# dropbox/lepton

Measured on NVIDIA H100. Metric: JPEG MB/s encode+decode, higher is better.
Workload: dtype int16 coefficients / u8 probabilities (integer)

## Files before the change

lepton_b200/csrc/lep_decode_g2.cu:

```cuda
#include "lep_common.cuh"
#include "lep_predict.cuh"

namespace lepb200 {

struct G2Bool {
    unsigned long long value;
    uint32_t range;
    int valid;
    uint32_t next;
    const uint8_t* p;
    const uint8_t* end;
};

__device__ __forceinline__ uint32_t g2_load_word(const uint8_t* p, const uint8_t* end) {
    uint32_t w = 0;
    const long long rem = end - p;
    if (rem > 0) {
        w = __byte_perm(__ldg(reinterpret_cast<const uint32_t*>(p)), 0u, 0x0123u);
        if (rem < 4) w &= 0xffffffffu << (8 * (4 - (int)rem));
    }
    return w;
}
__device__ __forceinline__ void g2_refill(G2Bool& r) {
    r.value |= (unsigned long long)r.next << (32 - r.valid);
    r.valid += 32;
    r.p += 4;
    r.next = g2_load_word(r.p, r.end);
}
__device__ __forceinline__ void g2_init(G2Bool& r, const uint8_t* p, uint32_t len) {
    r.value = 0; r.valid = 0; r.range = 255;
    r.p = p; r.end = p + len;
    r.next = g2_load_word(r.p, r.end);
    g2_refill(r);
    const uint32_t split = (r.range * 128u + 128u) >> 8;
    const uint32_t bit = (uint32_t)(r.value >> 56) >= split;
    const uint32_t range = bit ? r.range - split : split;
    if (bit) r.value -= (unsigned long long)split << 56;
    const int shift = __clz(range) - 24;
    r.range = range << shift; r.value <<= shift; r.valid -= shift;
}

__device__ __forceinline__ uint32_t g2_bit(G2Bool& r, const uint32_t* rcp, uint32_t w, uint32_t& split) {
    const uint32_t prob = branch_prob(w, rcp);
    split = (r.range * prob + (256 - prob)) >> 8;
    if (r.valid < 32) g2_refill(r);
    return (uint32_t)(r.value >> 56) >= split;
}
__device__ __forceinline__ void g2_update(G2Bool& r, uint32_t split, uint32_t bit) {
    const uint32_t range = bit ? r.range - split : split;
    if (bit) r.value -= (unsigned long long)split << 56;
    const int shift = __clz(range) - 24;
    r.range = range << shift;
    r.value <<= shift;
    r.valid -= shift;
}
__device__ __forceinline__ uint32_t g2_model_word(uint32_t w, uint32_t bit) {
    const bool plain = (w & 0xffu) < 254u && (w >> 8) < 254u;
    return (plain ? w + (bit ? 0x100u : 1u) : branch_update(w, bit)) & 0xffffu;
}
__device__ __forceinline__ uint32_t g2_get(G2Bool& r, uint16_t* model, const uint32_t* rcp, uint32_t addr, uint32_t w) {
    uint32_t split;
    const uint32_t bit = g2_bit(r, rcp, w, split);
    g2_update(r, split, bit);
    model[addr] = (uint16_t)g2_model_word(w, bit);
    return bit;
}
#ifdef LEPB200_EMU
#define G2_EMU_BARRIER() __syncwarp()
#else
#define G2_EMU_BARRIER()
#endif

__device__ __forceinline__ uint32_t g2_half8(uint4 v, uint32_t i) {
    const uint32_t u = (i & 4u) ? ((i & 2u) ? v.w : v.z) : ((i & 2u) ? v.y : v.x);
    return (u >> ((i & 1u) << 4)) & 0xffffu;
}
__device__ __forceinline__ uint32_t g2_half4(uint2 v, uint32_t i) {
    return (((i & 2u) ? v.y : v.x) >> ((i & 1u) << 4)) & 0xffffu;
}
__device__ __forceinline__ uint16_t& g2_gword(uint16_t* model, uint32_t width, uint32_t addr) { return model[mi_offset(addr, 0, width)]; }
__device__ __forceinline__ uint32_t g2_unit(const uint16_t* model, uint32_t width, uint32_t addr) {
    return *reinterpret_cast<const uint32_t*>(model + mi_offset(addr, 0, width));
}
__device__ __forceinline__ uint4 g2_units4(const uint16_t* model, uint32_t width, uint32_t addr) {
    return make_uint4(g2_unit(model, width, addr), g2_unit(model, width, addr + 2), g2_unit(model, width, addr + 4),
                      g2_unit(model, width, addr + 6));
}
struct G2NzTop { uint32_t r5, r4; uint2 r3; uint4 r2; };
__device__ __forceinline__ G2NzTop g2_nz_top(const uint16_t* top, const uint16_t* model, uint32_t width, uint32_t rear) {
    G2NzTop v;
    v.r5 = top[nz7_row(5) - nz7_row(3)];
    v.r4 = *reinterpret_cast<const uint32_t*>(top + (nz7_row(4) - nz7_row(3)));
    v.r3 = *reinterpret_cast<const uint2*>(top);
    v.r2 = g2_units4(model, width, rear + nz7_row(2));
    return v;
}
__device__ __forceinline__ uint16_t* g2_word(uint16_t* hot, uint16_t* model, uint32_t width, uint32_t addr) {
    return addr < M_HOT ? hot + addr : &g2_gword(model, width, addr);
}
struct G2EdgeTree { uint32_t r2, r1; uint2 r0; };
__device__ __forceinline__ G2EdgeTree g2_edge_tree(const uint16_t* model, uint32_t width, uint32_t t) {
    G2EdgeTree v;
    v.r2 = model[mi_offset(t + (2 << 2), 0, width)];
    v.r1 = g2_unit(model, width, t + (1 << 2));
    v.r0 = make_uint2(g2_unit(model, width, t), g2_unit(model, width, t + 2));
    return v;
}

enum : int { G2_EXP = 0, G2_SIGN = 1, G2_THR = 2, G2_RES = 3 };

struct alignas(16) G2GroupSmem {
    int16_t blk[4][64];
    int32_t tmp[64];
    int16_t pix[64];
    int16_t ledge[8];
};
static_assert(sizeof(G2GroupSmem) == 512 + 256 + 128 + 16, "group scratch layout");

template <int G> struct G2Cfg {
    static constexpr int S = 32 / G;
    static constexpr int WARPS = (G >= 4) ? 4 : G;
    static constexpr int THREADS = WARPS * 32;
    static constexpr size_t HOT_BYTES = (size_t)WARPS * S * M_HOT * 2;
    static constexpr size_t SMEM_BYTES = 512 * 4 + 64 + 64 + 2 * 52 * 4 + sizeof(G2GroupSmem) * WARPS * S + HOT_BYTES;
    static_assert(SMEM_BYTES <= 113 * 1024, "two CTAs of the group kernel per SM");
};

template <int G> __device__ __forceinline__ int g2_sum(int v) {
#pragma unroll
    for (int d = 1; d < G; d <<= 1) v += __shfl_xor_sync(FULL, v, d);
    return v;
}
template <int G> __device__ __forceinline__ int g2_min(int v) {
#pragma unroll
    for (int d = 1; d < G; d <<= 1) v = min(v, __shfl_xor_sync(FULL, v, d));
    return v;
}
template <int G> __device__ __forceinline__ int g2_max(int v) {
#pragma unroll
    for (int d = 1; d < G; d <<= 1) v = max(v, __shfl_xor_sync(FULL, v, d));
    return v;
}
template <int G> __device__ __forceinline__ uint32_t g2_or(uint32_t v) {
#pragma unroll
    for (int d = 1; d < G; d <<= 1) v |= __shfl_xor_sync(FULL, v, d);
    return v;
}

__device__ __forceinline__ uint32_t g2_edge_info(int prior, int min_thr) {
    const int bsr = bitlen((uint32_t)min(iabs(prior), 1023));
    const int p16 = (int)(int16_t)prior;
    const int sctx = p16 == 0 ? 0 : (p16 > 0 ? 1 : 2);
    const int ctx_abs = iabs(prior) & 0xffff;
    return (uint32_t)bsr | ((uint32_t)sctx << 4) | ((uint32_t)min_thr << 6) | ((uint32_t)min(ctx_abs >> min_thr, 255) << 9);
}

template <int G>
__global__ void __launch_bounds__(G2Cfg<G>::THREADS)
lep_decode_g2_kernel(const ImageDesc* __restrict__ images, SegDesc* __restrict__ segs, int first, int count, const int* __restrict__ order,
                     int* __restrict__ work_counter, uint16_t* __restrict__ model_pool, uint8_t* __restrict__ row_pool, size_t row_pool_stride) {
    constexpr int S = G2Cfg<G>::S;
    constexpr int CPL = 64 / G;
    __shared__ uint32_t s_rcp[512];
    __shared__ uint8_t s_a2r[64];
    __shared__ uint8_t s_nzbin[64];
    __shared__ uint32_t s_eb[2][52];
    __shared__ G2GroupSmem s_grp[G2Cfg<G>::WARPS * S];
#ifndef LEPB200_EMU
    extern __shared__ uint4 s_hot[];
#else
    static uint4 s_hot[G2Cfg<G>::HOT_BYTES / 16];
#endif
    for (int i = threadIdx.x; i < 512; i += blockDim.x) s_rcp[i] = i < 2 ? 0u : (uint32_t)((0x100000000ull + i - 1) / i);
    for (int i = threadIdx.x; i < 64; i += blockDim.x) { s_a2r[i] = c_aligned_to_raster[i]; s_nzbin[i] = i < 50 ? c_nonzero_to_bin[i] : 0; }
    for (int i = threadIdx.x; i < 2 * 52; i += blockDim.x) {
        const int cc = i / 52, n = i % 52;
        s_eb[cc][n] = m_exp7(cc, n < 50 ? c_nonzero_to_bin[n] : 0, 0, 0);
    }
    __syncthreads();
    const int lane = lane_id();
    const int sub = lane & (G - 1);
    const int gbase = lane & ~(G - 1);
    const int slot = (blockIdx.x * G2Cfg<G>::WARPS + (threadIdx.x >> 5)) * S + lane / G;
    G2GroupSmem& gs = s_grp[(threadIdx.x >> 5) * S + lane / G];
    uint4* const hot4 = s_hot + (size_t)((threadIdx.x >> 5) * S + lane / G) * (M_HOT / 8);
    uint16_t* const hot = reinterpret_cast<uint16_t*>(hot4);
    uint16_t* const eoff = reinterpret_cast<uint16_t*>(gs.tmp);
    uint32_t* const einfo = reinterpret_cast<uint32_t*>(gs.tmp) + 32;
    uint8_t* rowbuf = row_pool + (size_t)slot * row_pool_stride;

    bool alive = false;
    bool exhausted = false;
    SegDesc* sdp = nullptr;
    const ImageDesc* gp = images;
    uint16_t* model = model_pool;
    uint32_t mwidth = 1;
    int seg_min_y = 0, seg_max_y = 0;
    bool seg_last = false;
    G2Bool br;
    br.value = 0; br.valid = 0; br.range = 255; br.next = 0; br.p = nullptr; br.end = nullptr;
    unsigned long long ndec = 0;
    uint32_t top_mask = 7u, index = 0;
    int bw0 = 0, bw1 = 0, bw2 = 0, nzs0 = 0, nzs1 = 0;
    size_t nz_base = 0;
    int c = 0, ci = 0, y = 0, w = 0, x = 0, q0 = 1, pc = 0, pa = 2, nz_left = 0;
    bool has_above = false, need_row = true;
    int16_t* rowp = nullptr;
    const int16_t* abovep = nullptr;
    const uint16_t* q = nullptr;
    int16_t* redge = nullptr;
    uint8_t* rnz = nullptr;
    const int32_t* icx = nullptr;
    const int32_t* icy = nullptr;
    const uint8_t* mthr = nullptr;
    uint32_t cnt_top = 0, cnt_rear = 0;
    G2NzTop nzt = {};
    bool cnt_ready = false;

    for (;;) {
        const bool want_job = !alive && !exhausted;
        const unsigned claim = __ballot_sync(FULL, want_job && sub == 0);
        if (claim) {
            const int leader = __ffs(claim) - 1;
            int job0 = 0;
            if (lane == leader) job0 = atomicAdd(work_counter, __popc(claim));
            job0 = __shfl_sync(FULL, job0, leader);
            if (want_job) {
                const int job = job0 + __popc(claim & ((1u << gbase) - 1u));
                if (job >= count) {
                    exhausted = true;
                } else {
                    const int sidx = order[first + job];
                    sdp = &segs[sidx];
                    if (sdp->status == ST_OK) {
                        gp = &images[sdp->image];
                        model = model_pool + mi_model((size_t)job, (size_t)count);
                        mwidth = mi_width((size_t)job, (size_t)count);
                        seg_min_y = sdp->min_y; seg_max_y = sdp->max_y; seg_last = sdp->is_last != 0;
                        g2_init(br, reinterpret_cast<const uint8_t*>(sdp->stream), sdp->cap);
                        ndec = 0; top_mask = 7u; index = 0;
                        bw0 = gp->bch[0]; bw1 = gp->ncmp > 1 ? gp->bch[1] : 0; bw2 = gp->ncmp > 2 ? gp->bch[2] : 0;
                        nz_base = (size_t)(bw0 + bw1 + bw2) * 16;
                        nzs0 = (bw0 + 15) & ~15; nzs1 = (bw1 + 15) & ~15;
                        need_row = true;
                        alive = true;
                        for (int i = sub; i < (int)(M_HOT / 8); i += G) hot4[i] = make_uint4(0u, 0u, 0u, 0u);
                    }
                }
            }
        }
        if (alive && need_row) {
            const ImageDesc& g = *gp;
            for (;;) {
                const RowSpec rs = row_spec_from_index(index++, g);
                if (rs.done || (rs.luma_y >= seg_max_y && !seg_last)) { alive = false; break; }
                if (rs.skip || rs.luma_y < seg_min_y) continue;
                c = rs.component; y = rs.curr_y;
                has_above = !((top_mask >> c) & 1u);
                top_mask &= ~(1u << c);
                ci = c == 0 ? 0 : 1;
                w = g.bch[c];
                rowp = reinterpret_cast<int16_t*>(g.plane[c]) + (size_t)y * w * 64;
                abovep = rowp - (size_t)w * 64;
                q = g.q[c];
                q0 = q[0];
                redge = reinterpret_cast<int16_t*>(rowbuf + (size_t)(c == 0 ? 0 : (c == 1 ? bw0 : bw0 + bw1)) * 16);
                rnz = rowbuf + nz_base + (c == 0 ? 0 : (c == 1 ? nzs0 : nzs0 + nzs1));
                icx = g.icos_x[c];
                icy = g.icos_y[c];
                mthr = g.min_thr[c];
                x = 0; pc = 0; pa = 2; nz_left = 0;
                need_row = false;
                break;
            }
            if (!alive && sub == 0) {
                sdp->status = ST_OK;
                sdp->len = (uint32_t)(br.p - reinterpret_cast<const uint8_t*>(sdp->stream));
                sdp->ndecisions_lo = (uint32_t)ndec;
                sdp->ndecisions_hi = (uint32_t)(ndec >> 32);
            }
        }
        if (__all_sync(FULL, exhausted)) break;

        const bool has_left = x > 0;
        int16_t* rcur = gs.blk[pc];
        const int16_t* rleft = gs.blk[pc ^ 1];
        int16_t* rabove = gs.blk[pa];
        const int16_t* raleft = gs.blk[pa ^ 1];
        uint32_t nd = 0;
        int nz = 0;

        if (alive) {
            if (has_above) {
                const uint32_t* src = reinterpret_cast<const uint32_t*>(abovep + (size_t)x * 64) + sub * (CPL / 2);
#pragma unroll
                for (int k = 0; k < CPL / 2; ++k) {
                    const uint32_t u = src[k];
                    const int a = sub * CPL + 2 * k;
                    rabove[s_a2r[a]] = (int16_t)(u & 0xffff);
                    rabove[s_a2r[a + 1]] = (int16_t)(u >> 16);
                }
            }
#pragma unroll
            for (int k = 0; k < CPL / 2; ++k) reinterpret_cast<uint32_t*>(rcur)[sub * (CPL / 2) + k] = 0u;
        }
        __syncwarp();
        if (alive) {
            for (int zz = sub; zz < 49; zz += G) {
                const int coord = s_a2r[zz];
                uint32_t pr = 0;
                if (has_left && has_above) {
                    const uint32_t L = (uint32_t)iabs(rleft[coord]) & 0xffff, A = (uint32_t)iabs(rabove[coord]) & 0xffff;
                    pr = (((L + A) * 13u + (((uint32_t)iabs(raleft[coord]) & 0xffff) * 6u)) & 0xffff) >> 5;
                } else if (has_left || has_above) {
                    const int16_t nb = has_left ? rleft[coord] : rabove[coord];
                    pr = (uint32_t)iabs((int)(int16_t)((uint32_t)iabs(nb) & 0xffff));
                }
                eoff[zz] = (uint16_t)((zz * 12 + bitlen(min(pr, 1023u))) << 2);
            }
            if (!cnt_ready) {
                const int nz_above = has_above ? (int)rnz[x] : 0;
                int ctx = 0;
                if (has_above && !has_left) ctx = (nz_above + 1) / 2;
                else if (has_left && !has_above) ctx = (nz_left + 1) / 2;
                else if (has_left && has_above) ctx = (nz_above + nz_left + 2) / 4;
                cnt_top = m_nz7(ci, s_nzbin[ctx], 3, 0); cnt_rear = m_nz7(ci, s_nzbin[ctx], 0, 0);
                nzt = g2_nz_top(hot + cnt_top, model, mwidth, cnt_rear);
            }
        }
        cnt_ready = false;
        __syncwarp();

        {
            uint4 r1 = make_uint4(0u, 0u, 0u, 0u), r0 = r1;
            uint32_t prefix = 0;
#pragma unroll
            for (int idx = 5; idx >= 0; --idx) {
                const uint32_t mw = idx == 5 ? nzt.r5 : idx == 4 ? (nzt.r4 >> (prefix << 4)) & 0xffffu
                                  : idx == 3 ? g2_half4(nzt.r3, prefix) : idx == 2 ? g2_half8(nzt.r2, prefix)
                                  : idx == 1 ? g2_half8(r1, prefix & 7u) : g2_half8(r0, prefix & 7u);
                uint32_t split = 0, bit = 0;
                if (alive) bit = g2_bit(br, s_rcp, mw, split);
                const uint32_t p1 = (prefix << 1) | bit;
                if (alive && idx == 5) r1 = g2_units4(model, mwidth, cnt_rear + nz7_row(1) + (p1 << 3));
                if (alive && idx == 4) r0 = g2_units4(model, mwidth, cnt_rear + nz7_row(0) + (p1 << 3));
                if (idx >= 4) G2_EMU_BARRIER();
                if (alive) {
                    const uint16_t neww = (uint16_t)g2_model_word(mw, bit);
                    if (idx >= 3) hot[cnt_top + (nz7_row(idx) - nz7_row(3)) + prefix] = neww;
                    else g2_gword(model, mwidth, cnt_rear + nz7_row(idx) + prefix) = neww;
                    g2_update(br, split, bit);
                    prefix = p1;
                }
            }
            nz = (int)prefix;
            if (alive) nd += 6;
        }
        bool bad = false;
        if (alive && nz > 49) { bad = true; alive = false; }

        {
            int zz = 0, left_nz = nz, st = G2_EXP, len = 0, ri = 0, val = 0;
            bool neg = false;
            uint32_t addr = 0, a0 = 0, a1 = 0;
            bool busy = alive && nz > 0, b0 = busy, b1 = busy;
            const uint32_t sign_addr = m_sign(ci, 0, 0);
            if (busy) {
                const uint32_t eb = s_eb[ci][left_nz];
                addr = eb + eoff[0];
                a1 = addr + 1; a0 = eb + eoff[1];
            }
            uint32_t mw = busy ? *g2_word(hot, model, mwidth, addr) : 0u;
            while (__any_sync(FULL, busy)) {
                if (busy) {
                    uint32_t split;
                    const uint32_t bit = g2_bit(br, s_rcp, mw, split);
                    const uint32_t naddr = bit ? a1 : a0;
                    const bool nbusy = bit ? b1 : b0;
                    uint32_t mwn = nbusy ? *g2_word(hot, model, mwidth, naddr) : 0u;
                    const uint32_t neww = g2_model_word(mw, bit);
                    *g2_word(hot, model, mwidth, addr) = (uint16_t)neww;
                    if (naddr == addr) mwn = neww;
                    g2_update(br, split, bit);
                    ++nd;
                    const int isE = st == G2_EXP, isS = st == G2_SIGN, isR = st == G2_RES;
                    const int cont = isE & (int)bit & (int)(len < 10);
                    const int len1 = len + (isE & (int)bit);
                    const int ev0 = isE & (cont ^ 1) & (int)(len1 == 0);
                    const int toS = isE & (cont ^ 1) & (int)(len1 != 0);
                    const int ris = len - 2;
                    const int evS = isS & (int)(ris < 0), toR = isS & (int)(ris >= 0);
                    const int evR = isR & (int)(ri == 0);
                    const int evN = evS | evR, ev = ev0 | evN;
                    const int nval = isS ? (1 << ((len - 1) & 31)) : (isR ? (val | ((int)bit << (ri & 31))) : val);
                    const bool nneg = isS ? !bit : neg;
                    if (evN && sub == 0) rcur[s_a2r[zz]] = (int16_t)(nneg ? -nval : nval);
                    left_nz -= evN; zz += ev;
                    st = toS ? G2_SIGN : toR ? G2_RES : ev ? G2_EXP : st;
                    len = ev ? 0 : len1;
                    ri = isS ? ris : ri - isR;
                    val = nval; neg = nneg; addr = naddr; busy = nbusy; mw = mwn;
                    if (busy) {
                        const int zn = min(zz + 1, 48);
                        const bool lastpos = zz == 48;
                        const bool doneN = left_nz == 1 || lastpos;
                        const uint32_t nextN = s_eb[ci][left_nz - 1] + eoff[zn];
                        const bool inE = st == G2_EXP, inS = st == G2_SIGN;
                        const bool fin = inS ? len < 2 : ri == 0;
                        const uint32_t cont_a = inS ? m_resn(ci, s_a2r[zz], s_nzbin[left_nz]) + (uint32_t)(len - 2) : addr - 1;
                        const uint32_t common = fin ? nextN : cont_a;
                        const bool commonB = fin ? !doneN : true;
                        a1 = inE ? (len < 10 ? m_exp_next(addr, len) : sign_addr) : common;
                        a0 = inE ? (len == 0 ? s_eb[ci][left_nz] + eoff[zn] : sign_addr) : common;
                        b1 = inE ? true : commonB;
                        b0 = inE ? (len == 0 ? !lastpos : true) : commonB;
                    }
                }
            }
        }
        __syncwarp();

        int eobx = 0, eoby = 0;
        {
            uint32_t colmask = 0, rowmask = 0;
            if (alive) {
                for (int r = 1 + sub; r < 8; r += G) {
                    const uint4 u = *reinterpret_cast<const uint4*>(rcur + r * 8);
                    uint32_t m = 0;
                    m |= (u.x >> 16) ? 2u : 0u;
                    m |= (u.y & 0xffffu) ? 4u : 0u;   m |= (u.y >> 16) ? 8u : 0u;
                    m |= (u.z & 0xffffu) ? 16u : 0u;  m |= (u.z >> 16) ? 32u : 0u;
                    m |= (u.w & 0xffffu) ? 64u : 0u;  m |= (u.w >> 16) ? 128u : 0u;
                    colmask |= m;
                    if (m) rowmask |= 1u << r;
                }
            }
            colmask = g2_or<G>(colmask); rowmask = g2_or<G>(rowmask);
            eobx = colmask ? 31 - __clz(colmask) : 0;
            eoby = rowmask ? 31 - __clz(rowmask) : 0;
        }
        G2EdgeTree eth = {}, etv = {};
        if (alive) {
            eth = g2_edge_tree(model, mwidth, m_nze(0, ci, eobx, (nz + 3) / 7, 0, 0));
            etv = g2_edge_tree(model, mwidth, m_nze(1, ci, eoby, (nz + 3) / 7, 0, 0));
            for (int k = sub; k < 14; k += G) {
                int p = 0, coord;
                if (k < 7) { coord = k + 1; if (has_above) p = lak_pred(rcur, rabove, icx + (k + 1) * 8, k + 1, 8); }
                else { coord = 8 * (k - 6); if (has_left) p = lak_pred(rcur, rleft, icy + (k - 6) * 8, 8 * (k - 6), 1); }
                einfo[k] = g2_edge_info(p, mthr[coord]);
            }
        }
        __syncwarp();

#pragma unroll 1
        for (int vert = 0; vert < 2; ++vert) {
            int ne = 0;
            {
                const uint32_t base = m_nze(vert, ci, vert ? eoby : eobx, (nz + 3) / 7, 0, 0);
                const G2EdgeTree t = vert ? etv : eth;
                uint32_t prefix = 0;
#pragma unroll
                for (int idx = 2; idx >= 0; --idx) {
                    const uint32_t mw = idx == 2 ? t.r2 : idx == 1 ? (t.r1 >> (prefix << 4)) & 0xffffu : g2_half4(t.r0, prefix);
                    uint32_t split = 0, bit = 0;
                    if (alive) {
                        bit = g2_bit(br, s_rcp, mw, split);
                        g2_gword(model, mwidth, base + ((uint32_t)idx << 2) + prefix) = (uint16_t)g2_model_word(mw, bit);
                        g2_update(br, split, bit);
                        prefix = (prefix << 1) | bit;
                    }
                }
                ne = (int)prefix;
                if (alive) nd += 3;
            }
            int ln = 0, st = G2_EXP, len = 0, ri = 0, val = 0;
            bool neg = false;
            uint32_t addr = 0, e = 0, so = 1, thr_base = 0, a0 = 0, a1 = 0;
            const uint32_t expx_base = m_expx(ci, 0, vert * 7, 0);
            const uint32_t sign_base = m_sign(ci, 0, 0);
            const int cstep = vert ? 8 : 1;
            constexpr uint32_t NE_STRIDE = 15 * 12 * 4;
            constexpr uint32_t POS_STRIDE = 12 * 4;
            bool busy = alive && ne > 0, b0 = busy, b1 = busy;
            if (busy) {
                e = einfo[vert * 7];
                addr = expx_base + (uint32_t)ne * NE_STRIDE + ((e & 15u) << 2);
                a1 = addr + 1;
                a0 = expx_base + (uint32_t)ne * NE_STRIDE + POS_STRIDE + ((einfo[vert * 7 + 1] & 15u) << 2);
            }
            uint32_t mw = busy ? *g2_word(hot, model, mwidth, addr) : 0u;
            while (__any_sync(FULL, busy)) {
                if (busy) {
                    uint32_t split;
                    const uint32_t bit = g2_bit(br, s_rcp, mw, split);
                    const uint32_t naddr = bit ? a1 : a0;
                    const bool nbusy = bit ? b1 : b0;
                    uint32_t mwn = nbusy ? *g2_word(hot, model, mwidth, naddr) : 0u;
                    const uint32_t neww = g2_model_word(mw, bit);
                    *g2_word(hot, model, mwidth, addr) = (uint16_t)neww;
                    if (naddr == addr) mwn = neww;
                    g2_update(br, split, bit);
                    ++nd;
                    const int isE = st == G2_EXP, isS = st == G2_SIGN, isT = st == G2_THR, isR = st == G2_RES;
                    const int cont = isE & (int)bit & (int)(len < 10);
                    const int len1 = len + (isE & (int)bit);
                    const int ev0 = isE & (cont ^ 1) & (int)(len1 == 0);
                    const int toS = isE & (cont ^ 1) & (int)(len1 != 0);
                    const int mt = (int)((e >> 6) & 7u);
                    const int ris = len - 2;
                    const int evS = isS & (int)(ris < 0);
                    const int toT = isS & (int)(ris >= 0) & (int)(ris >= mt), toRs = isS & (int)(ris >= 0) & (int)(ris < mt);
                    const int rit = ri - 1;
                    const int evT = isT & (int)(ri == 0), toRt = isT & (int)(ri != 0) & (int)(rit < mt);
                    const int evR = isR & (int)(ri == 0);
                    const int evN = evS | evT | evR, ev = ev0 | evN;
                    const int nval = isS ? (1 << ((len - 1) & 31)) : ((isT | isR) ? (val | ((int)bit << (ri & 31))) : val);
                    const bool nneg = isS ? !bit : neg;
                    if (evN && sub == 0) rcur[(ln + 1) * cstep] = (int16_t)(nneg ? -nval : nval);
                    so = isT ? min((so << 1) | bit, 127u) : 1u;
                    thr_base = isS ? m_thr(ci, (int)((e >> 9) & 255u), min(len - mt, 7)) : thr_base;
                    ne -= evN; ln += ev;
                    if (ev) e = einfo[vert * 7 + min(ln, 6)];
                    st = toS ? G2_SIGN : toT ? G2_THR : (toRs | toRt) ? G2_RES : ev ? G2_EXP : st;
                    len = ev ? 0 : len1;
                    ri = isS ? ris : ri - (isT | isR);
                    val = nval; neg = nneg; addr = naddr; busy = nbusy; mw = mwn;
                    if (busy) {
                        const int mt2 = (int)((e >> 6) & 7u);
                        const bool lastpos = ln == 6;
                        const bool doneN = ne == 1 || lastpos;
                        const uint32_t nxt = (uint32_t)(ln + 1) * POS_STRIDE + ((einfo[vert * 7 + min(ln + 1, 6)] & 15u) << 2);
                        const uint32_t nextN = expx_base + (uint32_t)(ne - 1) * NE_STRIDE + nxt;
                        const uint32_t rb = m_resn(ci, (ln + 1) * cstep, ne);
                        const bool inE = st == G2_EXP, inS = st == G2_SIGN, inT = st == G2_THR;
                        const int r2 = inS ? len - 2 : ri - 1;
                        const bool fin = r2 < 0;
                        const bool thr = r2 >= mt2 && (inS || inT);
                        const uint32_t tb = inS ? m_thr(ci, (int)((e >> 9) & 255u), min(len - mt2, 7)) : thr_base;
                        const uint32_t so0 = inS ? 1u : min(so << 1, 127u), so1 = inS ? 1u : min((so << 1) | 1u, 127u);
                        const uint32_t rest = (inS || inT) ? rb + (uint32_t)r2 : addr - 1;
                        const uint32_t c0 = fin ? nextN : thr ? tb + so0 : rest;
                        const uint32_t c1 = fin ? nextN : thr ? tb + so1 : rest;
                        const bool cb = fin ? !doneN : true;
                        const uint32_t sa = sign_base + ((e >> 4) & 3u) * 12u + (e & 15u);
                        a1 = inE ? (len < 10 ? m_exp_next(addr, len) : sa) : c1;
                        a0 = inE ? (len == 0 ? expx_base + (uint32_t)ne * NE_STRIDE + nxt : sa) : c0;
                        b1 = inE ? true : cb;
                        b0 = inE ? (len == 0 ? !lastpos : true) : cb;
                    }
                }
            }
        }
        __syncwarp();

        if (alive) {
            for (int r = sub; r < 8; r += G) {
                int32_t in[8], out[8];
#pragma unroll
                for (int k = 0; k < 8; ++k) in[k] = (int32_t)rcur[r * 8 + k] * (int32_t)q[r * 8 + k];
                if (r == 0) in[0] = 0;
                idct_row(in, out);
#pragma unroll
                for (int k = 0; k < 8; ++k) gs.tmp[r * 8 + k] = out[k];
            }
        }
        __syncwarp();
        if (alive) {
            for (int col = sub; col < 8; col += G) {
                int32_t in[8], out[8];
#pragma unroll
                for (int k = 0; k < 8; ++k) in[k] = gs.tmp[k * 8 + col];
                idct_col(in, out);
#pragma unroll
                for (int k = 0; k < 8; ++k) gs.pix[k * 8 + col] = (int16_t)out[k];
            }
        }
        __syncwarp();
        int pred = 0;
        uint32_t dc_exp = 0, dc_sign = 0, dc_res = 0;
        {
            int sl = 0, sa = 0, mnl = 32767, mxl = -32768, mna = 32767, mxa = -32768;
            if (alive) {
                for (int i = sub; i < 16; i += G) {
                    if (i < 8) {
                        if (has_left) {
                            const int16_t p0 = gs.pix[i * 8], p1 = gs.pix[i * 8 + 1];
                            const int16_t delta = (int16_t)(p0 - p1);
                            const int est = (int16_t)((int16_t)((int16_t)gs.ledge[i] - half_rz16(delta)) - (int16_t)(p0 + 1024));
                            sl += est; mnl = min(mnl, est); mxl = max(mxl, est);
                        }
                    } else if (has_above) {
                        const int j = i - 8;
                        const int16_t p0 = gs.pix[j], p1 = gs.pix[8 + j];
                        const int16_t delta = (int16_t)(p0 - p1);
                        const int est = (int16_t)((int16_t)((int16_t)redge[(size_t)x * 8 + j] - half_rz16(delta)) - (int16_t)(p0 + 1024));
                        sa += est; mna = min(mna, est); mxa = max(mxa, est);
                    }
                }
            }
            sl = g2_sum<G>(sl); sa = g2_sum<G>(sa);
            mnl = g2_min<G>(mnl); mna = g2_min<G>(mna);
            mxl = g2_max<G>(mxl); mxa = g2_max<G>(mxa);
            if (alive) {
                int avgmed = 0, unc = 0, unc2 = 0;
                if (has_left || has_above) {
                    int a0, a1, mn_all, mx_all;
                    if (has_left && has_above) { a0 = sl; a1 = sa; mn_all = min(mnl, mna); mx_all = max(mxl, mxa); }
                    else if (has_left) { a0 = a1 = sl; mn_all = mnl; mx_all = mxl; }
                    else { a0 = a1 = sa; mn_all = mna; mx_all = mxa; }
                    avgmed = (a0 + a1) >> 1;
                    unc = (mx_all - mn_all) >> 3;
                    a0 -= avgmed; a1 -= avgmed;
                    int far_afield = a1;
                    if (iabs(a0) < iabs(a1)) far_afield = a0;
                    unc2 = far_afield >> 3;
                }
                pred = (div_trunc_small(avgmed, q0) + 4) >> 3;
                const int lm = min(bitlen((uint32_t)iabs(unc) & 0xffff), 11), lo16 = min(bitlen((uint32_t)iabs(unc2) & 0xffff), 16);
                const int sctx = unc2 >= 0 ? (unc2 == 0 ? 3 : 2) : 1;
                dc_exp = m_expdc(lm, lo16); dc_sign = m_sign(ci, 0, sctx); dc_res = m_resdc(lm);
            }
        }

        int dcv = 0;
        {
            int st = G2_EXP, len = 0, ri = 0, val = 0;
            bool neg = false;
            uint32_t addr = dc_exp, a0 = dc_exp, a1 = dc_exp + 1;
            bool busy = alive, b0 = false, b1 = busy;
            uint32_t mw = busy ? *g2_word(hot, model, mwidth, addr) : 0u;
            while (__any_sync(FULL, busy)) {
                if (busy) {
                    uint32_t split;
                    const uint32_t bit = g2_bit(br, s_rcp, mw, split);
                    const uint32_t naddr = bit ? a1 : a0;
                    const bool nbusy = bit ? b1 : b0;
                    uint32_t mwn = nbusy ? *g2_word(hot, model, mwidth, naddr) : 0u;
                    const uint32_t neww = g2_model_word(mw, bit);
                    *g2_word(hot, model, mwidth, addr) = (uint16_t)neww;
                    if (naddr == addr) mwn = neww;
                    g2_update(br, split, bit);
                    ++nd;
                    const int isE = st == G2_EXP, isS = st == G2_SIGN, isR = st == G2_RES;
                    const int cont = isE & (int)bit & (int)(len < 10);
                    const int len1 = len + (isE & (int)bit);
                    const int toS = isE & (cont ^ 1) & (int)(len1 != 0);
                    const int ris = len - 2;
                    const int evS = isS & (int)(ris < 0), toR = isS & (int)(ris >= 0);
                    const int evR = isR & (int)(ri == 0);
                    const int nval = isS ? (1 << ((len - 1) & 31)) : (isR ? (val | ((int)bit << (ri & 31))) : val);
                    const bool nneg = isS ? !bit : neg;
                    if (evS | evR) dcv = nneg ? -nval : nval;
                    st = toS ? G2_SIGN : toR ? G2_RES : st;
                    len = len1;
                    ri = isS ? ris : ri - isR;
                    val = nval; neg = nneg; addr = naddr; busy = nbusy; mw = mwn;
                    if (busy) {
                        const bool inE = st == G2_EXP, inS = st == G2_SIGN;
                        const bool fin = inS ? len < 2 : ri == 0;
                        const uint32_t common = inS ? dc_res + (uint32_t)(len - 2) : addr - 1;
                        a1 = inE ? (len < 10 ? m_exp_next(addr, len) : dc_sign) : common;
                        a0 = inE ? dc_sign : common;
                        b1 = inE ? true : !fin;
                        b0 = inE ? len != 0 : !fin;
                    }
                }
            }
        }

        if (alive) {
            const int dc = (int)(int16_t)adv_unpredict((int)(int16_t)dcv, true, pred);
            if (sub == 0) rcur[0] = (int16_t)dc;
            const int16_t qdc = (int16_t)((uint32_t)q0 * (uint32_t)dc);
            for (int i = sub; i < 16; i += G) {
                if (i < 8) {
                    const int16_t cur = gs.pix[i * 8 + 7], prev = gs.pix[i * 8 + 6];
                    const int16_t delta = (int16_t)(cur - prev);
                    gs.ledge[i] = (int16_t)(cur + half_rz16(delta) + 1024 + qdc);
                } else {
                    const int j = i - 8;
                    const int16_t cur = gs.pix[56 + j], prev = gs.pix[48 + j];
                    const int16_t delta = (int16_t)(cur - prev);
                    redge[(size_t)x * 8 + j] = (int16_t)(cur + half_rz16(delta) + 1024 + qdc);
                }
            }
            if (sub == 0) rnz[x] = (uint8_t)nz;
            nz_left = nz;
        }
        ndec += nd;
        if (bad) {
            if (sub == 0) {
                sdp->status = ST_STREAM_INCONSISTENT;
                sdp->len = (uint32_t)(br.p - reinterpret_cast<const uint8_t*>(sdp->stream));
                sdp->ndecisions_lo = (uint32_t)ndec;
                sdp->ndecisions_hi = (uint32_t)(ndec >> 32);
            }
        }
        __syncwarp();
        if (alive) {
            uint32_t* dst = reinterpret_cast<uint32_t*>(rowp + (size_t)x * 64) + sub * (CPL / 2);
#pragma unroll
            for (int k = 0; k < CPL / 2; ++k) {
                const int a = sub * CPL + 2 * k;
                const uint32_t lo = (uint16_t)rcur[s_a2r[a]];
                const uint32_t hi = (uint16_t)rcur[s_a2r[a + 1]];
                dst[k] = lo | (hi << 16);
            }
            if (x + 1 >= w || (uint32_t)((size_t)y * w + x + 1) >= (uint32_t)gp->trunc_bc[c]) {
                need_row = true;
            } else {
                const int nza = has_above ? (int)rnz[x + 1] : 0;
                const int bin = s_nzbin[has_above ? (nza + nz + 2) / 4 : (nz + 1) / 2];
                cnt_top = m_nz7(ci, bin, 3, 0); cnt_rear = m_nz7(ci, bin, 0, 0);
                nzt = g2_nz_top(hot + cnt_top, model, mwidth, cnt_rear);
                cnt_ready = true;
                ++x; pc ^= 1; pa ^= 1;
            }
        }
        __syncwarp();
    }
}

}
```

Before: 696.8.

## Tune group decode kernel: occupancy bounds, packed shuffles, static first-wave jobs, vector copies

Adds a minBlocksPerSM launch bound tied to group size, so the compiler limits registers and more CTAs fit per SM. Packs the min/max and column/row-mask shuffle reductions into paired 16-bit lanes, halving the number of warp shuffles. The first job of each slot is assigned statically, skipping one atomic per group at startup. Row reads and writes go through 128-bit vector copies when the width allows. The tighter register cap may cause spills, and the static first wave assumes the work counter starts after the grid's slot count.

```diff
diff --git a/lepton_b200/csrc/lep_decode_g2.cu b/lepton_b200/csrc/lep_decode_g2.cu
--- a/lepton_b200/csrc/lep_decode_g2.cu
+++ b/lepton_b200/csrc/lep_decode_g2.cu
@@ -122,8 +122,10 @@
     static constexpr int WARPS = (G >= 4) ? 4 : G;
     static constexpr int THREADS = WARPS * 32;
     static constexpr size_t HOT_BYTES = (size_t)WARPS * S * M_HOT * 2;
+    static constexpr int CTAS = G == 8 ? 4 : G == 4 ? 2 : 1;
     static constexpr size_t SMEM_BYTES = 512 * 4 + 64 + 64 + 2 * 52 * 4 + sizeof(G2GroupSmem) * WARPS * S + HOT_BYTES;
-    static_assert(SMEM_BYTES <= 113 * 1024, "two CTAs of the group kernel per SM");
+    static_assert(G != 4 || SMEM_BYTES <= 113 * 1024, "two CTAs of the group kernel per SM at G = 4");
+    static_assert(G != 8 || SMEM_BYTES <= 56 * 1024, "four CTAs of the group kernel per SM at G = 8");
 };
 
 template <int G> __device__ __forceinline__ int g2_sum(int v) {
@@ -131,20 +133,32 @@
     for (int d = 1; d < G; d <<= 1) v += __shfl_xor_sync(FULL, v, d);
     return v;
 }
-template <int G> __device__ __forceinline__ int g2_min(int v) {
-#pragma unroll
-    for (int d = 1; d < G; d <<= 1) v = min(v, __shfl_xor_sync(FULL, v, d));
-    return v;
-}
-template <int G> __device__ __forceinline__ int g2_max(int v) {
-#pragma unroll
-    for (int d = 1; d < G; d <<= 1) v = max(v, __shfl_xor_sync(FULL, v, d));
+__device__ __forceinline__ uint32_t g2_vminu2(uint32_t a, uint32_t b) {
+#ifdef LEPB200_EMU
+    return std::min(a & 0xffffu, b & 0xffffu) | (std::min(a >> 16, b >> 16) << 16);
+#else
+    return __vminu2(a, b);
+#endif
+}
+template <int G> __device__ __forceinline__ uint32_t g2_min2(uint32_t v) {
+#pragma unroll
+    for (int d = 1; d < G; d <<= 1) v = g2_vminu2(v, __shfl_xor_sync(FULL, v, d));
     return v;
 }
 template <int G> __device__ __forceinline__ uint32_t g2_or(uint32_t v) {
 #pragma unroll
     for (int d = 1; d < G; d <<= 1) v |= __shfl_xor_sync(FULL, v, d);
     return v;
+}
+
+template <int N> __device__ __forceinline__ void g2_copy_words(uint32_t* dst, const uint32_t* src) {
+    if constexpr (N % 4 == 0) {
+#pragma unroll
+        for (int k = 0; k < N; k += 4) *reinterpret_cast<uint4*>(dst + k) = *reinterpret_cast<const uint4*>(src + k);
+    } else {
+#pragma unroll
+        for (int k = 0; k < N; ++k) dst[k] = src[k];
+    }
 }
 
 __device__ __forceinline__ uint32_t g2_edge_info(int prior, int min_thr) {
@@ -156,7 +170,7 @@
 }
 
 template <int G>
-__global__ void __launch_bounds__(G2Cfg<G>::THREADS)
+__global__ void __launch_bounds__(G2Cfg<G>::THREADS, G2Cfg<G>::CTAS)
 lep_decode_g2_kernel(const ImageDesc* __restrict__ images, SegDesc* __restrict__ segs, int first, int count, const int* __restrict__ order,
                      int* __restrict__ work_counter, uint16_t* __restrict__ model_pool, uint8_t* __restrict__ row_pool, size_t row_pool_stride) {
     constexpr int S = G2Cfg<G>::S;
@@ -191,6 +205,7 @@
 
     bool alive = false;
     bool exhausted = false;
+    bool first_wave = true;
     SegDesc* sdp = nullptr;
     const ImageDesc* gp = images;
     uint16_t* model = model_pool;
@@ -223,8 +238,12 @@
         if (claim) {
             const int leader = __ffs(claim) - 1;
             int job0 = 0;
-            if (lane == leader) job0 = atomicAdd(work_counter, __popc(claim));
-            job0 = __shfl_sync(FULL, job0, leader);
+            if (first_wave) job0 = slot - lane / G;
+            else {
+                if (lane == leader) job0 = (int)gridDim.x * (G2Cfg<G>::WARPS * S) + atomicAdd(work_counter, __popc(claim));
+                job0 = __shfl_sync(FULL, job0, leader);
+            }
+            first_wave = false;
             if (want_job) {
                 const int job = job0 + __popc(claim & ((1u << gbase) - 1u));
                 if (job >= count) {
@@ -292,7 +311,8 @@
 
         if (alive) {
             if (has_above) {
-                const uint32_t* src = reinterpret_cast<const uint32_t*>(abovep + (size_t)x * 64) + sub * (CPL / 2);
+                uint32_t src[CPL / 2];
+                g2_copy_words<CPL / 2>(src, reinterpret_cast<const uint32_t*>(abovep + (size_t)x * 64) + sub * (CPL / 2));
 #pragma unroll
                 for (int k = 0; k < CPL / 2; ++k) {
                     const uint32_t u = src[k];
@@ -435,7 +455,8 @@
                     if (m) rowmask |= 1u << r;
                 }
             }
-            colmask = g2_or<G>(colmask); rowmask = g2_or<G>(rowmask);
+            const uint32_t masks = g2_or<G>(colmask | (rowmask << 8));
+            colmask = masks & 0xffu; rowmask = masks >> 8;
             eobx = colmask ? 31 - __clz(colmask) : 0;
             eoby = rowmask ? 31 - __clz(rowmask) : 0;
         }
@@ -599,8 +620,12 @@
                 }
             }
             sl = g2_sum<G>(sl); sa = g2_sum<G>(sa);
-            mnl = g2_min<G>(mnl); mna = g2_min<G>(mna);
-            mxl = g2_max<G>(mxl); mxa = g2_max<G>(mxa);
+            {
+                const uint32_t mn = g2_min2<G>((uint32_t)(mnl + 32768) | ((uint32_t)(mna + 32768) << 16));
+                const uint32_t mx = g2_min2<G>((uint32_t)(32767 - mxl) | ((uint32_t)(32767 - mxa) << 16));
+                mnl = (int)(mn & 0xffffu) - 32768; mna = (int)(mn >> 16) - 32768;
+                mxl = 32767 - (int)(mx & 0xffffu); mxa = 32767 - (int)(mx >> 16);
+            }
             if (alive) {
                 int avgmed = 0, unc = 0, unc2 = 0;
                 if (has_left || has_above) {
@@ -698,14 +723,15 @@
         }
         __syncwarp();
         if (alive) {
-            uint32_t* dst = reinterpret_cast<uint32_t*>(rowp + (size_t)x * 64) + sub * (CPL / 2);
+            uint32_t out[CPL / 2];
 #pragma unroll
             for (int k = 0; k < CPL / 2; ++k) {
                 const int a = sub * CPL + 2 * k;
                 const uint32_t lo = (uint16_t)rcur[s_a2r[a]];
                 const uint32_t hi = (uint16_t)rcur[s_a2r[a + 1]];
-                dst[k] = lo | (hi << 16);
-            }
+                out[k] = lo | (hi << 16);
+            }
+            g2_copy_words<CPL / 2>(reinterpret_cast<uint32_t*>(rowp + (size_t)x * 64) + sub * (CPL / 2), out);
             if (x + 1 >= w || (uint32_t)((size_t)y * w + x + 1) >= (uint32_t)gp->trunc_bc[c]) {
                 need_row = true;
             } else {
```

Measured after the change: 698.3, median of 6. Within noise of the previous version (+0.2%).
